# eric612/Mobilenet-YOLO-Pytorch

Hardware: AMD Instinct MI355X
Metric: images/sec MobileNetV2-YOLO 352x352 fwd+bwd @ bs256 (higher is better)
Workload: dtype f32; 1 GPU; MobileNetV2-YOLO 352x352 bs=256/GPU fwd+loss+bwd fp32 (BASELINE configs[1]); global_batch=256, parallelism=dp1

## Files before the change

### mobilenet-yolo-pytorch_amd/csrc/pwgemm.hip

```cpp
#include <map>
#include <mutex>

#include "pwgemm.h"
#include "x6.h"
#include "pwnt_kernel.h"

namespace mny {

static Nt2Kernel nt2_kernel(int TN, int XF, int BF = 0, int RED = 0, int X6 = 0, int RB = 0) {
    if (RED) return nt2_red_kernel(TN, XF, BF, RED, X6, RB);
#define MNY_K(T, XF_, BF_, RED_, X6_, RB_) case nt2_key(T, XF_, BF_, RED_, X6_, RB_): return (Nt2Kernel)pw_gemm_nt_dma_kernel<T, XF_, BF_, RED_, X6_, RB_>;
#define MNY_FWD(T, BF_, X6_) MNY_K(T, 0, BF_, 0, X6_, 0) MNY_K(T, 1, BF_, 0, X6_, 0) MNY_K(T, 2, BF_, 0, X6_, 0)
#define MNY_TN5(M_, ...) M_(1, __VA_ARGS__) M_(2, __VA_ARGS__) M_(3, __VA_ARGS__) M_(4, __VA_ARGS__) M_(5, __VA_ARGS__)
    switch (nt2_key(TN, XF, BF, RED, X6, RB)) {
        MNY_TN5(MNY_FWD, 0, 0) MNY_TN5(MNY_FWD, 0, 1) MNY_TN5(MNY_FWD, 0, 3) MNY_TN5(MNY_FWD, 1, 0)
    }
#undef MNY_TN5
#undef MNY_FWD
#undef MNY_K
    return nullptr;
}

struct Nt2Plan { int TN, n_tiles, m_tiles, gx, tiles_per_block, grid; size_t lds; };

// ... 14 lines not shown
    const Cut3Job jb = jobs[block_job[blockIdx.x]];
    const int nk = (jb.C + 15) / 16;
    const int64_t idx = (int64_t)(blockIdx.x - jb.block0) * 256 + threadIdx.x;
    if (idx >= (int64_t)jb.R * nk * 2) return;
    const int h = (int)(idx & 1);
    const int64_t rk = idx >> 1;
    const int kt = (int)(rk % nk);
    const int64_t row = rk / nk;
    float x[8];
#pragma unroll
    for (int e = 0; e < 8; ++e) {
        const int k = kt * 16 + (e < 4 ? 4 * h + e : 8 + 4 * h + (e - 4));
        x[e] = k < jb.C ? jb.src[row * jb.C + k] : 0.f;
    }
    bf16x8_t hh, mm, ll;
    x6_split(v4f_t{x[0], x[1], x[2], x[3]}, v4f_t{x[4], x[5], x[6], x[7]}, hh, mm, ll);
    const int64_t plane = (int64_t)jb.R * nk * 32;
    char* d = reinterpret_cast<char*>(jb.dst) + idx * 16;
    *reinterpret_cast<v4f_t*>(d) = __builtin_bit_cast(v4f_t, hh);
    *reinterpret_cast<v4f_t*>(d + plane) = __builtin_bit_cast(v4f_t, mm);
    *reinterpret_cast<v4f_t*>(d + 2 * plane) = __builtin_bit_cast(v4f_t, ll);
}

static int nt2_blocks_per_cu(int TN, int XF, size_t lds, int BF = 0) {
    static std::map<uint64_t, int> cache;
    static std::mutex mu;
    const uint64_t key = ((uint64_t)BF << 48) | ((uint64_t)TN << 40) | ((uint64_t)XF << 32) | (uint64_t)lds;
    std::lock_guard<std::mutex> lock(mu);
    auto it = cache.find(key);
    if (it != cache.end()) return it->second;
    int nb = 0;
    if (hipOccupancyMaxActiveBlocksPerMultiprocessor(&nb, (const void*)nt2_kernel(TN, XF, BF), 256, lds) != hipSuccess || nb < 1) nb = 1;
    if (nb > 8) nb = 8;
    cache[key] = nb;
    return nb;
}

static Nt2Plan nt2_plan(int64_t M, int K, int N, bool xf, int BF = 0, int tn_cap = 5) {
    Nt2Plan pl;
    int best = 1, best_pad = 1 << 30;
    for (int tn = tn_cap; tn >= 1; --tn) {
        int pad = (int)cdiv(N, 32 * tn) * 32 * tn;
        if (pad < best_pad) { best_pad = pad; best = tn; }
    }
    const int blocks_per_cu = nt2_blocks_per_cu(best, 1, nt2_lds(best, K, true, BF), BF);
    pl.TN = best;
    pl.n_tiles = (int)cdiv(N, 32 * best);
    pl.m_tiles = (int)cdiv(M, BM);
    int want = 256 * blocks_per_cu / pl.n_tiles;
    if (want < 8) want = 8;
    if (want > kMaxParts) want = kMaxParts;
    int gx = pl.m_tiles < want ? pl.m_tiles : want;
    pl.tiles_per_block = (int)cdiv(pl.m_tiles, gx);
    constexpr double min_ai = 100.0;
    const double ai = 2.0 * K * N / ((BF ? 2.0 : 4.0) * (K + N));
    if (ai >= min_ai) {
        const int t_min = pl.tiles_per_block;
        long best_cost = -1;
        int best_t = t_min, best_b = 0;
        for (int t = t_min; t <= 4 * t_min + 4 && t <= pl.m_tiles; ++t) {
            const int g = (int)cdiv(pl.m_tiles, t);
            const int nb = g * pl.n_tiles;
            if (nb < 256) break;
            const long cost = (long)cdiv(nb, 256) * t;
            if (best_cost < 0 || cost < best_cost || (cost == best_cost && nb > best_b)) { best_cost = cost; best_t = t; best_b = nb; }
        }
        pl.tiles_per_block = best_t;
    }
    pl.gx = (int)cdiv(pl.m_tiles, pl.tiles_per_block);
    pl.grid = (int)cdiv(pl.gx, 8) * 8 * pl.n_tiles;
    pl.lds = nt2_lds(best, K, xf, BF);
    return pl;
}

template <typename T>
__global__ void transpose_kernel(const float* __restrict__ src, T* __restrict__ dst, int R, int Cc, int Rp) {
    __shared__ float tile[32][33];
    const int bx = blockIdx.x * 32, by = blockIdx.y * 32;
    for (int j = threadIdx.y; j < 32; j += 8) {
        const int r = by + j, c = bx + threadIdx.x;
        tile[j][threadIdx.x] = (r < R && c < Cc) ? src[(int64_t)r * Cc + c] : 0.f;
    }
    __syncthreads();
    for (int j = threadIdx.y; j < 32; j += 8) {
        const int c = bx + j, r = by + threadIdx.x;
        if (r < Rp && c < Cc) st1(dst + (int64_t)c * Rp + r, r < R ? tile[threadIdx.x][j] : 0.f);
    }
}

}

using namespace mny;
static thread_local int g_pw_route = -1;
void mny::pw_set_last_route(int family) { g_pw_route = family; }

struct PwRoute {
    int family = MNY_ROUTE_TILE_V1;
    const char* why = nullptr;
    int parts = MNY_EINVAL;
    bool as_counted = true;
    int64_t Mf = 0;
    int wide_parts = 0;
    int x6 = 0;
    Nt2Plan p2{};
    size_t lds = 0;
};

static bool w6_pays(int K, int Nc) {
    constexpr double min_ai = 30.0;
    return !sw(SW_NO_W6) && 2.0 * K * Nc / (4.0 * (K + Nc)) >= min_ai;
}

static PwRoute pw_fwd_route(int bf, int64_t M, int K, int Nc, int in_act, bool view, bool bias, bool addend, bool planes) {
    PwRoute r;
    if (M <= 0 || K <= 0 || Nc <= 0) { r.why = "empty problem"; return r; }
    const bool v1 = sw(SW_GEMM_V1);
    const bool thin = pw_thin_ok(bf, 0, M, K, Nc);
    const bool wide = !bf && !thin && pw_wide_ok(M, K, Nc, false);
    auto family = [&](int act, bool has_bias, bool has_addend) {
        if (bf && pwt_ok(M, K, Nc, act, has_bias)) return MNY_ROUTE_WAVE16;
        if (thin) return MNY_ROUTE_THIN;
        if (wide && !has_bias && !has_addend && act != MNY_ACT_HSIGMOID) return MNY_ROUTE_WIDE;
        if ((K & (bf ? 7 : 3)) || v1) return MNY_ROUTE_TILE_V1;
        return !bf && nt_x6(M, K, Nc) ? MNY_ROUTE_DMA_X6 : MNY_ROUTE_DMA_F32;
    };
    r.family = family(in_act, bias, addend);
    const int plain = in_act == MNY_ACT_NONE && !bias && !addend ? r.family : family(MNY_ACT_NONE, false, false);
    r.as_counted = r.family == plain;
    if (planes && (bf || plain != MNY_ROUTE_DMA_X6 || pw_wide_ok(M, K, Nc, true) || !w6_pays(K, Nc))) r.why = "no pre-cut weight planes for this problem (mny_pw_w6_supported)";
    const bool xf = view || in_act != MNY_ACT_NONE;
    switch (r.family) {
        case MNY_ROUTE_WAVE16: r.parts = pwt_parts(M); return r;
        case MNY_ROUTE_THIN: r.parts = pw_thin_parts(M, K, Nc, 0); return r;
        case MNY_ROUTE_TILE_V1: r.parts = pw_v1_parts(M, K, Nc); return r;
        case MNY_ROUTE_WIDE:
            r.Mf = M & ~(int64_t)31;
            r.parts = r.wide_parts = pw_wide_parts(M, K, Nc, false);
            if (r.Mf == M) return r;
            r.p2 = nt2_plan(M - r.Mf, K, Nc, xf);
            r.x6 = nt_x6(M, K, Nc);
            r.parts += r.p2.gx;
            break;
        default:
            r.p2 = nt2_plan(M, K, Nc, xf, bf);
            r.x6 = r.family == MNY_ROUTE_DMA_X6;
            r.parts = r.p2.gx;
    }
    r.lds = r.p2.lds;
    size_t lds_max = 64 * 1024;
    if (planes) {
        r.x6 = 3;
#if MNY_W6_SWP
        r.lds = (size_t)(3 * BM * 16 + 3 * 32 * r.p2.TN * 24) * sizeof(float) + (xf ? 2 * cdiv(K, 16) * 16 * sizeof(float) : 0);
#endif
        lds_max = 96 * 1024;
    }
    if (!r.why && r.lds > lds_max) r.why = "K too large for the LDS scale cache";
    return r;
}

constexpr int kRedMaxTn = 4;
static PwRoute pw_dgrad_bnred_route(int bf, int64_t M, int K, int Nc, int act, bool addend, bool planes) {
    PwRoute r;
    if (M <= 0 || K <= 0 || Nc <= 0 || (K & (bf ? 7 : 3))) { r.why = "empty problem, or dy rows that are not 16-byte aligned"; return r; }
    const bool v1 = sw(SW_GEMM_V1), thin32 = pw_thin_ok(0, 1, M, K, Nc), wide = pw_wide_ok(M, K, Nc, true);
    r.x6 = !bf && nt_x6(M, K, Nc);
    bool tile = false;
    if (bf && pwt_ok(M, K, Nc, MNY_ACT_NONE, false)) {
        r.family = MNY_ROUTE_WAVE16;
        r.parts = pwt_parts(M);
    } else if (bf ? pw_thin_ok(1, 1, M, K, Nc) : thin32) {
        r.family = MNY_ROUTE_THIN;
        r.parts = pw_thin_parts(M, K, Nc, 1);
    } else if (!bf && wide) {
        r.family = MNY_ROUTE_WIDE;
        r.Mf = M & ~(int64_t)31;
        r.parts = r.wide_parts = pw_wide_parts(M, K, Nc, true);
        if (r.Mf != M) {
            r.p2 = nt2_plan(M - r.Mf, K, Nc, false, 0, kRedMaxTn);
            r.parts += r.p2.gx;
        }
    } else {
        r.family = v1 ? MNY_ROUTE_TILE_V1 : r.x6 ? MNY_ROUTE_DMA_X6 : MNY_ROUTE_DMA_F32;
        r.p2 = nt2_plan(M, K, Nc, false, bf, kRedMaxTn);
        r.parts = r.p2.gx;
        tile = true;
    }
    r.lds = r.p2.lds;
    if (act < MNY_ACT_NONE || act > MNY_ACT_HSIGMOID) r.why = "unknown activation";
    else if (v1) r.why = "MNY_GEMM_V1 is set";
    else if (K >= 512 && Nc >= 512) r.why = "matrix-pipe-bound: the reduce pass it would save is cheaper than the longer epilogue";
    else if (thin32 && act == MNY_ACT_HSIGMOID) r.why = "the short-reduction kernel knows the clamp family and h-swish (what units use)";
    else if (wide && act >= MNY_ACT_HSWISH) r.why = "the wide-output kernel's reduction form knows the clamp family (its h-swish builds spill)";
    else if (addend && tile && r.p2.TN > 3) r.why = "the addend form needs a column tile of <= 96 (mny_pw_dgrad_bnred_add_supported)";
    else if (planes && (bf || r.family != MNY_ROUTE_DMA_X6 || pw_wide_ok(M, K, Nc, false) || !w6_pays(K, Nc))) r.why = "no pre-cut weight planes for this problem (mny_pw_w6_supported)";
    else if (r.lds > (size_t)(planes ? 96 : 64) * 1024) r.why = "K too large";
    if (planes) r.x6 = 3;
    return r;
}

static PwRoute pw_lr_fix_route(int64_t M, int K, int r_act, bool red, bool view) {
    PwRoute r;
    if (M <= 0 || K <= 0 || (K & 3)) { r.why = "empty problem, or rows that are not 16-byte aligned"; return r; }
    if (red && pw_wide_fix_ok(M, K) && r_act < MNY_ACT_HSWISH) {
        r.family = MNY_ROUTE_WIDE;
        r.parts = pw_wide_fix_parts(M, K);
        return r;
    }
    r.p2 = nt2_plan(M, K, K, view, 0, 3);
    r.lds = r.p2.lds;
    r.x6 = nt_x6(M, K, K);
    r.family = r.x6 ? MNY_ROUTE_DMA_X6 : MNY_ROUTE_DMA_F32;
    r.parts = r.p2.gx;
    if (r.lds > 64 * 1024) r.why = "K too large";
    return r;
}

extern "C" int mny_pw_stat_parts(int64_t M, int K, int Nc) { return pw_fwd_route(0, M, K, Nc, MNY_ACT_NONE, false, false, false, false).parts; }
extern "C" int mny_pw_stat_parts_bf16(int64_t M, int K, int Nc) { return pw_fwd_route(1, M, K, Nc, MNY_ACT_NONE, false, false, false, false).parts; }

static int nt2_launch(const PwRoute& r, int XF, int BF, int RED, int RB, const Gemm2Args& g, hipStream_t st, const char* what) {
    const Nt2Kernel k = nt2_kernel(r.p2.TN, XF, BF, RED, r.x6, RB);
    if (!k) {
        set_error("%s: no kernel for a %d-column tile", what, 32 * r.p2.TN); return MNY_EUNSUPPORTED;
    }
    nt2_allow_lds(k, r.lds);
    hipLaunchKernelGGL(k, dim3(r.p2.grid), dim3(256), r.lds, st, g);
    return check_launch(what);
}

template <int BF>
static int pw_fwd_impl(const void* x, const float* in_scale, const float* in_shift, int in_act, const void* w, const float* bias, const void* addend,
                       void* y, float* stats, int64_t M, int K, int Nc, void* stream, bool planes = false) {
    MNY_REQUIRE(x && w && y, "pw_fwd: null pointer");
    MNY_REQUIRE(!(stats && bias), "pw_fwd: stats and bias are mutually exclusive");
    const PwRoute r = pw_fwd_route(BF, M, K, Nc, in_act, in_scale != nullptr, bias != nullptr, addend != nullptr, planes);
    MNY_REQUIRE(!r.why, "pw_fwd: M=%lld K=%d N=%d: %s", (long long)M, K, Nc, r.why);
    MNY_REQUIRE(!stats || r.as_counted, "pw_fwd: statistics with in_act=%d%s%s at M=%lld K=%d N=%d take another kernel family than mny_pw_stat_parts%s counted rows for",
                in_act, bias ? ", a bias" : "", addend ? ", an addend" : "", (long long)M, K, Nc, BF ? "_bf16" : "");
    g_pw_route = r.family;
    hipStream_t st = (hipStream_t)stream;
    switch (r.family) {
        case MNY_ROUTE_WAVE16: return pwt_launch(x, in_scale, in_shift, in_act, w, addend, y, stats, M, K, Nc, st);
        case MNY_ROUTE_THIN:
            return pw_thin_launch(BF, x, in_scale, in_shift, in_act, w, bias, addend, y, stats, M, K, Nc, 0, nullptr, nullptr, nullptr, nullptr, nullptr, 0, st);
        case MNY_ROUTE_TILE_V1: return pw_v1_launch(BF, x, in_scale, in_shift, in_act, w, bias, addend, y, stats, M, K, Nc, st);
        case MNY_ROUTE_WIDE: {
            const int rc = pw_wide_launch((const float*)x, in_scale, in_shift, in_act, (const float*)w, (float*)y, stats, r.Mf, K, Nc, nullptr, nullptr, nullptr, nullptr,
                                          nullptr, 0, nullptr, st);
            if (rc != 0 || r.Mf == M) return rc;
            if (stats) stats += (int64_t)r.wide_parts * 2 * Nc;
            x = (const float*)x + r.Mf * K; y = (float*)y + r.Mf * Nc; M -= r.Mf;
        }
    }
    Gemm2Args g{x, in_scale, in_shift, in_act, w, bias, addend, y, stats, M, K, Nc, r.p2.m_tiles, r.p2.tiles_per_block, r.p2.gx, r.p2.n_tiles,
                nullptr, nullptr, nullptr, nullptr, nullptr, 0};
    const int XF = !in_scale && in_act == MNY_ACT_NONE ? 0 : (in_act == MNY_ACT_HSWISH ? 2 : 1);
    return nt2_launch(r, XF, BF, 0, 0, g, st, "pw_gemm_nt_dma_kernel");
}
extern "C" int mny_pw_fwd(const float* x, const float* in_scale, const float* in_shift, int in_act, const float* w,
                          const float* bias, const float* addend, float* y, float* stats, int64_t M, int K, int Nc,
                          void* stream) {
    return pw_fwd_impl<0>(x, in_scale, in_shift, in_act, w, bias, addend, y, stats, M, K, Nc, stream);
}
extern "C" int mny_pw_fwd_bf16(const void* x, const float* in_scale, const float* in_shift, int in_act, const void* w,
                               const float* bias, const void* addend, void* y, float* stats, int64_t M, int K, int Nc,
                               void* stream) {
    return pw_fwd_impl<1>(x, in_scale, in_shift, in_act, w, bias, addend, y, stats, M, K, Nc, stream);
}

template <int BF>
static int pw_dgrad_bnred_impl(const void* dy, const void* wT, void* dx, const void* y, const float* scale, const float* shift, int act,
                               const float* mean, const float* invstd, float* red, int64_t M, int K, int Nc, void* stream, const void* addend = nullptr,
                               bool planes = false) {
    MNY_REQUIRE(dy && wT && dx && y && scale && shift && mean && invstd && red, "pw_dgrad_bnred: null pointer");
    const PwRoute r = pw_dgrad_bnred_route(BF, M, K, Nc, act, addend != nullptr, planes);
    MNY_REQUIRE(!r.why, "pw_dgrad_bnred: unsupported problem M=%lld K=%d N=%d act=%d: %s (see mny_pw_dgrad_bnred_supported)", (long long)M, K, Nc, act, r.why);
    g_pw_route = r.family;
    hipStream_t st = (hipStream_t)stream;
    switch (r.family) {
        case MNY_ROUTE_WAVE16: return pwt_launch(dy, nullptr, nullptr, MNY_ACT_NONE, wT, addend, dx, red, M, K, Nc, st, y, scale, shift, mean, invstd, act);
        case MNY_ROUTE_THIN:
            return pw_thin_launch(BF, dy, nullptr, nullptr, MNY_ACT_NONE, wT, nullptr, addend, dx, red, M, K, Nc, addend ? 2 : 1, y, scale, shift, mean, invstd, act, st);
        case MNY_ROUTE_WIDE: {
            const int rc = pw_wide_launch((const float*)dy, nullptr, nullptr, MNY_ACT_NONE, (const float*)wT, (float*)dx, red, r.Mf, K, Nc, (const float*)y, scale, shift,
                                          mean, invstd, act, (const float*)addend, st);
            if (rc != 0 || r.Mf == M) return rc;
            red += (int64_t)r.wide_parts * 2 * Nc;
            dy = (const float*)dy + r.Mf * K; dx = (float*)dx + r.Mf * Nc; y = (const float*)y + r.Mf * Nc;
            if (addend) addend = (const float*)addend + r.Mf * Nc;
            M -= r.Mf;
        }
    }
    Gemm2Args g{dy, nullptr, nullptr, MNY_ACT_NONE, wT, nullptr, addend, dx, red, M, K, Nc, r.p2.m_tiles, r.p2.tiles_per_block, r.p2.gx, r.p2.n_tiles,
                y, scale, shift, mean, invstd, act};
    return nt2_launch(r, 0, BF, addend ? 2 : 1, 0, g, st, "pw_gemm_nt_dma_kernel<RED>");
}
extern "C" int mny_pw_dgrad_bnred_supported(int64_t M, int K, int Nc, int act) { return !pw_dgrad_bnred_route(0, M, K, Nc, act, false, false).why; }
extern "C" int mny_pw_dgrad_bnred_parts(int64_t M, int K, int Nc) { return pw_dgrad_bnred_route(0, M, K, Nc, MNY_ACT_NONE, false, false).parts; }
extern "C" int mny_pw_dgrad_bnred(const float* dy, const float* wT, float* dx, const float* y, const float* scale, const float* shift, int act,
                                  const float* mean, const float* invstd, float* red, int64_t M, int K, int Nc, void* stream) {
    return pw_dgrad_bnred_impl<0>(dy, wT, dx, y, scale, shift, act, mean, invstd, red, M, K, Nc, stream);
}
extern "C" int mny_pw_dgrad_bnred_add_supported(int64_t M, int K, int Nc, int act) { return !pw_dgrad_bnred_route(0, M, K, Nc, act, true, false).why; }
extern "C" int mny_pw_dgrad_bnred_add_supported_bf16(int64_t M, int K, int Nc, int act) { return !pw_dgrad_bnred_route(1, M, K, Nc, act, true, false).why; }
extern "C" int mny_pw_dgrad_bnred_add(const float* dy, const float* wT, const float* addend, float* dx, const float* y, const float* scale, const float* shift,
// ... 113 lines not shown
```

### mobilenet-yolo-pytorch_amd/csrc/pwnt_kernel.h

```cpp
#pragma once
#include <type_traits>

#include "common.h"
#include "dma_zero.h"
#include "x6.h"

namespace mny {

constexpr int BM = 128;

struct Gemm2Args {
    const void* A; const float* in_scale; const float* in_shift; int in_act;
    const void* B; const float* bias; const void* addend; void* C; float* stats;
    int64_t M; int K; int N;
    int m_tiles, tiles_per_block, gx, n_tiles;
    const void* rY; const float* r_scale; const float* r_shift; const float* r_mean; const float* r_invstd; int r_act;
};

#ifndef MNY_W6_GROUP
#define MNY_W6_GROUP 4
#endif
#ifndef MNY_W6_SWP
#define MNY_W6_SWP 1
#endif
template <int TN, int XF, int BF, int RED = 0, int X6 = 0, int RB = 0>
__global__ __launch_bounds__(256) __attribute__((amdgpu_waves_per_eu((X6 == 3 && RED == 0 && MNY_W6_SWP) ? 2 : 3, 8))) void pw_gemm_nt_dma_kernel(Gemm2Args p) {
    using T = typename std::conditional<BF != 0, bf16_t, float>::type;
    constexpr int EPC = BF ? 8 : 4;
    constexpr int BKE = 4 * EPC;
    const T* pA = (const T*)p.A;
    const T* pB = (const T*)p.B;
    const T* pAdd = (const T*)p.addend;
    T* pC = (T*)p.C;
    constexpr int BN = 32 * TN, BKD = 16, S = 3;
    constexpr int A_ST = BM * BKD, B_ST = X6 == 3 ? BN * 24 : BN * BKD;
    constexpr int NA = BM / 16, NB = X6 == 3 ? 3 * TN : BN / 16, NL = NA + NB;
    constexpr int LPW = (NL + 3) / 4;
    constexpr bool SWP = X6 == 3 && RED == 0 && MNY_W6_SWP != 0;
    constexpr int SB = X6 == 3 ? (SWP ? 3 : 2) : S;
    constexpr int NA_W = NA / 4;
    static_assert(NA % 4 == 0 && NA_W < LPW, "slot split");
    extern __shared__ __attribute__((aligned(16))) float smem[];
    float* const sA = smem;
    float* const sB = smem + S * A_ST;
    float* sScale = sB + SB * B_ST;

    const int bid = blockIdx.x, xcd = bid & 7, local = bid >> 3;
    const int y = local % p.n_tiles, x = (local / p.n_tiles) * 8 + xcd;
    if (x >= p.gx) return;
    const int n0 = y * BN;

    const int tid = threadIdx.x, lane = tid & 63;
    const int wv = __builtin_amdgcn_readfirstlane(tid >> 6);
    const int lrow = lane & 31, khalf = lane >> 5;
    const int swz = (lrow >> 2) & 3;
    const int nk = (p.K + BKE - 1) / BKE;
    const int Kpad = nk * BKE;
    float* sShift = sScale + Kpad;
    const float slope = act_slope(p.in_act), hi = act_hi(p.in_act);
    if (XF != 0) {
        const bool has_xf = p.in_scale != nullptr;
        for (int k = tid; k < Kpad; k += 256) {
            sScale[k] = (k < p.K) ? (has_xf ? p.in_scale[k] : 1.f) : 0.f;
            sShift[k] = (k < p.K && has_xf) ? p.in_shift[k] : 0.f;
        }
    }
    const int mt_begin = x * p.tiles_per_block;
    const int mt_end = min(mt_begin + p.tiles_per_block, p.m_tiles);
    const int total = (mt_end - mt_begin) * nk;

    const int drow = lane >> 2;
    const int dk = ((lane & 3) ^ ((drow >> 2) & 3)) * EPC;
    int d_lds[LPW], d_row0[LPW];
    bool d_isA[LPW];
    const T* d_bptr[LPW];
#pragma unroll
    for (int i = 0; i < LPW; ++i) {
        int j = wv + 4 * i;
        if (j >= NL) j = NL - 1;
        d_isA[i] = j < NA;
        d_row0[i] = (d_isA[i] ? j : j - NA) * 16;
        d_lds[i] = d_isA[i] ? j * 256 : (j - NA) * 256;
        if constexpr (X6 == 3) {
            const int jb = d_isA[i] ? 0 : j - NA;
            const int pl = jb / TN, u = jb - pl * TN;
            int n = n0 + u * 32 + (lane & 31);
            if (n >= p.N) n = p.N - 1;
            d_lds[i] = d_isA[i] ? j * 256 : jb * 256;
            d_bptr[i] = reinterpret_cast<const T*>(reinterpret_cast<const char*>(p.B) + ((int64_t)pl * p.N + n) * nk * 32 + (lane >> 5) * 16);
        } else {
            int n = n0 + d_row0[i] + drow;
            if (n >= p.N) n = p.N - 1;
            d_bptr[i] = pB + (int64_t)n * p.K + dk;
        }
    }
    const T* zero_src = reinterpret_cast<const T*>(&mny_zero16);
    const bool ragged_k = (p.K % BKE) != 0;

    const T* d_cur[LPW];
    int d_step[LPW];
#pragma unroll
    for (int i = 0; i < LPW; ++i) d_step[i] = d_isA[i] ? BKE : (X6 == 3 ? 32 / (int)sizeof(T) : BKE);
    auto seat = [&](int mt) {
#pragma unroll
        for (int i = 0; i < LPW; ++i) {
            if (d_isA[i]) {
                int m = mt * BM + d_row0[i] + drow;
                if (m >= (int)p.M) m = (int)p.M - 1;
                d_cur[i] = pA + (int64_t)m * p.K + dk;
            } else {
                d_cur[i] = d_bptr[i];
            }
        }
    };
    auto issue_part = [&](int kt, float* stage, int i0, int i1) {
#pragma unroll
        for (int i = 0; i < LPW; ++i) {
            if (i < i0 || i >= i1) continue;
            const T* src = d_cur[i];
            if (ragged_k) {
                const bool kout = kt == nk - 1 && kt * BKE + dk >= p.K;
                if (kout) src = d_isA[i] ? d_cur[i] - (kt * BKE + dk) : (X6 == 3 ? src : zero_src);
            }
            d_cur[i] += d_step[i];
            __builtin_amdgcn_global_load_lds((const __attribute__((address_space(1))) void*)src,
                                             (__attribute__((address_space(3))) void*)(stage + d_lds[i]), 16, 0, 0);
        }
    };
    auto issue_a = [&](int kt, int slot) { issue_part(kt, sA + slot * A_ST, 0, NA_W); };
    auto issue_b = [&](int kt, int slot) { issue_part(kt, sB + slot * B_ST, NA_W, LPW); };

    f32x16 acc[TN];
#pragma unroll
    for (int t = 0; t < TN; ++t)
#pragma unroll
        for (int r = 0; r < 16; ++r) acc[t][r] = 0.f;
    float s1[TN], s2[TN];
#pragma unroll
    for (int t = 0; t < TN; ++t) { s1[t] = 0.f; s2[t] = 0.f; }

    auto compute = [&](int kt, int slot, int slot_b) {
        const float* stA = sA + slot * A_ST;
        const float* stB = sB + slot_b * B_ST;
        const float* a_row = stA + (wv * 32 + lrow) * BKD;
        if constexpr (BF != 0) {
#pragma unroll
            for (int kc = 0; kc < 2; ++kc) {
                const int chunk = kc * 2 + khalf;
                v4u_t au = lds_read_u4(a_row + ((chunk ^ swz) << 2));
                v4u_t bu[TN];
#pragma unroll
                for (int u = 0; u < TN; ++u) bu[u] = lds_read_u4(stB + (u * 32 + lrow) * BKD + ((chunk ^ swz) << 2));
                v4f_t sc0, sc1, sh0, sh1;
                if (XF != 0) {
                    const int kbase = kt * BKE + chunk * 8;
                    sc0 = lds_read_f4(sScale + kbase); sc1 = lds_read_f4(sScale + kbase + 4);
                    sh0 = lds_read_f4(sShift + kbase); sh1 = lds_read_f4(sShift + kbase + 4);
                }
                MNY_LGKM_WAIT(au);
#pragma unroll
                for (int u = 0; u < TN; ++u) MNY_LGKM_DEP(bu[u]);
                if (XF != 0) {
                    MNY_LGKM_DEP(sc0); MNY_LGKM_DEP(sc1); MNY_LGKM_DEP(sh0); MNY_LGKM_DEP(sh1);
                    float z[8] = {__uint_as_float(au.x << 16), __uint_as_float(au.x & 0xffff0000u), __uint_as_float(au.y << 16),
                                  __uint_as_float(au.y & 0xffff0000u), __uint_as_float(au.z << 16), __uint_as_float(au.z & 0xffff0000u),
                                  __uint_as_float(au.w << 16), __uint_as_float(au.w & 0xffff0000u)};
                    const float scv[8] = {sc0.x, sc0.y, sc0.z, sc0.w, sc1.x, sc1.y, sc1.z, sc1.w};
                    const float shv[8] = {sh0.x, sh0.y, sh0.z, sh0.w, sh1.x, sh1.y, sh1.z, sh1.w};
#pragma unroll
                    for (int e = 0; e < 8; ++e) {
                        const float zz = fmaf(z[e], scv[e], shv[e]);
                        z[e] = XF == 1 ? __builtin_amdgcn_fmed3f(zz, slope * zz, hi) : zz * __builtin_amdgcn_fmed3f(zz + 3.f, 0.f, 6.f) * (1.f / 6.f);
                    }
                    au = v4u_t{pack_bf16x2(z[0], z[1]), pack_bf16x2(z[2], z[3]), pack_bf16x2(z[4], z[5]), pack_bf16x2(z[6], z[7])};
                }
                const bf16x8_t a8 = __builtin_bit_cast(bf16x8_t, au);
// ... 93 lines not shown
                    af.x = z0 * fminf(fmaxf(z0 + 3.f, 0.f), 6.f) * (1.f / 6.f); af.y = z1 * fminf(fmaxf(z1 + 3.f, 0.f), 6.f) * (1.f / 6.f);
                    af.z = z2 * fminf(fmaxf(z2 + 3.f, 0.f), 6.f) * (1.f / 6.f); af.w = z3 * fminf(fmaxf(z3 + 3.f, 0.f), 6.f) * (1.f / 6.f);
                }
            }
#pragma unroll
            for (int u = 0; u < TN; ++u) acc[u] = __builtin_amdgcn_mfma_f32_32x32x2f32(af.x, bf[u].x, acc[u], 0, 0, 0);
#pragma unroll
            for (int u = 0; u < TN; ++u) acc[u] = __builtin_amdgcn_mfma_f32_32x32x2f32(af.y, bf[u].y, acc[u], 0, 0, 0);
#pragma unroll
            for (int u = 0; u < TN; ++u) acc[u] = __builtin_amdgcn_mfma_f32_32x32x2f32(af.z, bf[u].z, acc[u], 0, 0, 0);
#pragma unroll
            for (int u = 0; u < TN; ++u) acc[u] = __builtin_amdgcn_mfma_f32_32x32x2f32(af.w, bf[u].w, acc[u], 0, 0, 0);
        }
    };

    const int quad = lrow >> 2, jq = lane & 3;
    const bool nvec = (p.N & 3) == 0;
    auto epilogue = [&](int mt) {
        const int64_t m0 = (int64_t)mt * BM;
#pragma unroll
        for (int u = 0; u < TN; ++u) {
            const int colq = n0 + u * 32 + quad * 4;
            const bool cok = colq < p.N;
            float4 bv = f4zero();
            if (p.bias && cok) {
                if (nvec) bv = ld4(p.bias + colq);
                else {
                    bv.x = p.bias[colq];
                    if (colq + 1 < p.N) bv.y = p.bias[colq + 1];
                    if (colq + 2 < p.N) bv.z = p.bias[colq + 2];
                    if (colq + 3 < p.N) bv.w = p.bias[colq + 3];
                }
            }
            if (RED) {
                const int col = n0 + u * 32 + lrow;
                const bool ccol = col < p.N;
                const int cc = ccol ? col : 0;
                const float rsc = p.r_scale[cc], rsh = p.r_shift[cc], rmu = p.r_mean[cc], ris = p.r_invstd[cc];
                float rbias = 0.f;
                if constexpr (RB != 0) rbias = p.bias[cc];
                const float rslope = act_slope(p.r_act), rhi = act_hi(p.r_act);
                const int64_t rbase = m0 + wv * 32 + 4 * khalf;
                const int rows_left = (int)max((int64_t)0, min((int64_t)64, p.M - rbase));
                const T* ybase = (const T*)p.rY + (rows_left > 0 ? rbase : 0) * p.N + cc;
                const T* abase = RED == 2 ? pAdd + (rows_left > 0 ? rbase : 0) * p.N + cc : nullptr;
#pragma unroll
                for (int gq = 0; gq < 4; ++gq) {
                    float yv[4], av[4] = {0.f, 0.f, 0.f, 0.f};
#pragma unroll
                    for (int j = 0; j < 4; ++j) yv[j] = ld1(ybase + (ccol && 8 * gq + j < rows_left ? 8 * gq + j : 0) * p.N);
                    if (RED == 2) {
#pragma unroll
                        for (int j = 0; j < 4; ++j) av[j] = ld1(abase + (ccol && 8 * gq + j < rows_left ? 8 * gq + j : 0) * p.N);
                    }
#pragma unroll
                    for (int j = 0; j < 4; ++j) {
                        const float z = fmaf(yv[j], rsc, rsh);
                        const float dact = p.r_act >= MNY_ACT_HSWISH ? act_bwd(z, p.r_act) : (z > 0.f ? 1.f : rslope) * (z < rhi ? 1.f : 0.f);
                        const float dz = stored<T>(RB != 0 ? acc[u][gq * 4 + j] + rbias + av[j] : acc[u][gq * 4 + j] + av[j]) * dact;
                        if (ccol && 8 * gq + j < rows_left) { s1[u] += dz; s2[u] = fmaf(dz, (yv[j] - rmu) * ris, s2[u]); }
                    }
                    __builtin_amdgcn_sched_barrier(0);
                }
            } else if (p.stats) {
                const bool ccol = n0 + u * 32 + lrow < p.N;
                if (m0 + BM <= p.M) {
                    v2f a1 = v2f{0.f, 0.f}, a2 = v2f{0.f, 0.f};
#pragma unroll
                    for (int r = 0; r < 16; r += 2) {
                        const v2f q = v2f{stored<T>(acc[u][r]), stored<T>(acc[u][r + 1])};
                        a1 += q;
                        a2 = __builtin_elementwise_fma(q, q, a2);
                    }
                    if (ccol) { s1[u] += a1.x + a1.y; s2[u] += a2.x + a2.y; }
                } else {
#pragma unroll
                    for (int r = 0; r < 16; ++r) {
                        const int64_t row = m0 + wv * 32 + (r & 3) + 8 * (r >> 2) + 4 * khalf;
                        const float q = stored<T>(acc[u][r]);
                        if (ccol && row < p.M) { s1[u] += q; s2[u] = fmaf(q, q, s2[u]); }
                    }
                }
            }
#pragma unroll
            for (int gq = 0; gq < 4; ++gq) {
                float r0 = acc[u][gq * 4 + 0], r1 = acc[u][gq * 4 + 1], r2 = acc[u][gq * 4 + 2], r3 = acc[u][gq * 4 + 3];
                {
                    const bool odd = lane & 1;
                    const float xa = odd ? r0 : r1, xb = odd ? r2 : r3;
                    const float ya = __builtin_bit_cast(float, __builtin_amdgcn_mov_dpp(__builtin_bit_cast(int, xa), 0xB1, 0xF, 0xF, true));
                    const float yb = __builtin_bit_cast(float, __builtin_amdgcn_mov_dpp(__builtin_bit_cast(int, xb), 0xB1, 0xF, 0xF, true));
                    if (odd) { r0 = ya; r2 = yb; } else { r1 = ya; r3 = yb; }
                }
                {
                    const bool hi2 = lane & 2;
                    const float xa = hi2 ? r0 : r2, xb = hi2 ? r1 : r3;
                    const float ya = __builtin_bit_cast(float, __builtin_amdgcn_mov_dpp(__builtin_bit_cast(int, xa), 0x4E, 0xF, 0xF, true));
                    const float yb = __builtin_bit_cast(float, __builtin_amdgcn_mov_dpp(__builtin_bit_cast(int, xb), 0x4E, 0xF, 0xF, true));
                    if (hi2) { r0 = ya; r1 = yb; } else { r2 = ya; r3 = yb; }
                }
                const int64_t row = m0 + wv * 32 + 8 * gq + 4 * khalf + jq;
                if (cok && row < p.M) {
                    float4 v = make_float4(r0, r1, r2, r3);
                    if (p.bias) { v.x += bv.x; v.y += bv.y; v.z += bv.z; v.w += bv.w; }
                    if (nvec) {
                        if (pAdd) add4(v, ld4(pAdd + row * p.N + colq));
                        if (sizeof(T) == 2) st4(pC + row * p.N + colq, v); else st4_stream(pC + row * p.N + colq, v);
                    } else {
                        T* dst = pC + row * p.N + colq;
                        const T* ad = pAdd ? pAdd + row * p.N + colq : nullptr;
                        st1(dst, v.x + (ad ? ld1(ad) : 0.f));
                        if (colq + 1 < p.N) st1(dst + 1, v.y + (ad ? ld1(ad + 1) : 0.f));
                        if (colq + 2 < p.N) st1(dst + 2, v.z + (ad ? ld1(ad + 2) : 0.f));
                        if (colq + 3 < p.N) st1(dst + 3, v.w + (ad ? ld1(ad + 3) : 0.f));
                    }
                }
#pragma unroll
                for (int i = 0; i < 4; ++i) acc[u][gq * 4 + i] = 0.f;
                __builtin_amdgcn_sched_barrier(0);
            }
        }
    };

    int c_mt = mt_begin, c_kt = 0, c_slot = 0, c_slot_b = 0;
    auto consume = [&]() {
        compute(c_kt, c_slot, X6 != 3 ? c_slot : c_slot_b);
        if (++c_kt == nk) { epilogue(c_mt); c_kt = 0; ++c_mt; }
        if (++c_slot == S) c_slot = 0;
        c_slot_b ^= 1;
    };
    if constexpr (X6 != 3) {
        int i_mt = mt_begin, i_kt = 0, i_slot = 0;
        seat(mt_begin);
        auto issue_next = [&]() {
            issue_a(i_kt, i_slot); issue_b(i_kt, i_slot);
            if (++i_kt == nk) { i_kt = 0; ++i_mt; if (i_mt < mt_end) seat(i_mt); }
            if (++i_slot == S) i_slot = 0;
        };
        const int pre = total < S - 1 ? total : S - 1;
        for (int t = 0; t < pre; ++t) issue_next();
        const int steady = total - pre;
        for (int t = 0; t < steady; ++t) {
            wait_vmcnt<LPW*(S - 2)>();
            __builtin_amdgcn_s_barrier();
            issue_next();
            consume();
        }
        for (int t = 0; t < pre; ++t) {
            wait_vmcnt<0>();
            __builtin_amdgcn_s_barrier();
            consume();
        }
    } else if constexpr (SWP) {
        int a_mt = mt_begin, a_kt = 0, a_slot = 0, a_n = 0;
        int b_mt = mt_begin, b_kt = 0, b_slot = 0, b_n = 0;
        auto seat_part = [&](int mt, bool part_a) {
#pragma unroll
            for (int i = 0; i < LPW; ++i) {
                if ((i < NA_W) != part_a) continue;
                if (part_a) {
                    int m = mt * BM + d_row0[i] + drow;
                    if (m >= (int)p.M) m = (int)p.M - 1;
                    d_cur[i] = pA + (int64_t)m * p.K + dk;
                } else {
                    d_cur[i] = d_bptr[i];
                }
            }
        };
        seat_part(mt_begin, true); seat_part(mt_begin, false);
        auto next_a = [&]() {
            issue_a(a_kt, a_slot); ++a_n;
            if (++a_kt == nk) { a_kt = 0; ++a_mt; if (a_mt < mt_end) seat_part(a_mt, true); }
            if (++a_slot == S) a_slot = 0;
        };
        auto next_b = [&]() {
            issue_b(b_kt, b_slot); ++b_n;
            if (++b_kt == nk) { b_kt = 0; ++b_mt; if (b_mt < mt_end) seat_part(b_mt, false); }
            if (++b_slot == SB) b_slot = 0;
        };
        const unsigned oA0 = lds_off(sA + (wv * 32 + lrow) * BKD + ((khalf ^ swz) << 2));
        const unsigned oA1 = lds_off(sA + (wv * 32 + lrow) * BKD + (((2 + khalf) ^ swz) << 2));
        const unsigned oB = lds_off(sB + lane * 4);
        const unsigned oS = lds_off(sScale + khalf * 4);
        const unsigned shift_off = (unsigned)Kpad * 4u;
        bf16x8_t qh, qm, ql;
        int p_kt = 0, p_slot = 0;
        int m_slot_b = 0;
        auto step = [&](auto prep_c, auto mma_c) -> bool {
            constexpr bool PREP = decltype(prep_c)::value, MMA = decltype(mma_c)::value;
            constexpr int NPIECE = 24, NISSUE = MMA ? 6 * TN : 1;
            v4f_t a0, a1, sc0, sc1, sh0, sh1;
            float z[8];
            v2f r1[4], r2[4];
            v4u_t nhu, nmu, nlu;
            auto piece = [&](auto pc) {
                constexpr int P = decltype(pc)::value;
                if constexpr (PREP) {
                    if constexpr (P < 8) {
                        const float av = P < 4 ? a0[P & 3] : a1[P & 3];
                        if constexpr (XF != 0) {
                            const float zz = fmaf(av, P < 4 ? sc0[P & 3] : sc1[P & 3], P < 4 ? sh0[P & 3] : sh1[P & 3]);
                            z[P] = XF == 1 ? __builtin_amdgcn_fmed3f(zz, slope * zz, hi) : zz * __builtin_amdgcn_fmed3f(zz + 3.f, 0.f, 6.f) * (1.f / 6.f);
                        } else {
                            z[P] = av;
                        }
                        asm volatile("" : "+v"(z[P]));
                    } else if constexpr (P < 16) {
                        constexpr int i = (P - 8) >> 1;
                        if constexpr (((P - 8) & 1) == 0) {
                            const v2f a = v2f{z[2 * i], z[2 * i + 1]};
                            const v2f ah = v2f{__uint_as_float(__float_as_uint(a.x) & 0xffff0000u), __uint_as_float(__float_as_uint(a.y) & 0xffff0000u)};
                            r1[i] = a - ah;
                            asm volatile("" : "+v"(r1[i]));
                        } else {
                            const v2f b = r1[i];
                            const v2f bh = v2f{__uint_as_float(__float_as_uint(b.x) & 0xffff0000u), __uint_as_float(__float_as_uint(b.y) & 0xffff0000u)};
                            r2[i] = b - bh;
                            asm volatile("" : "+v"(r2[i]));
                        }
                    } else if constexpr (P < 22) {
                        constexpr int q = P - 16, w = q >> 1, d = (q & 1) * 2;
                        auto pk = [](float lo, float hi_) { return __builtin_amdgcn_perm(__float_as_uint(hi_), __float_as_uint(lo), 0x07060302u); };
                        unsigned t0, t1;
                        if constexpr (w == 0) { t0 = pk(z[2 * d], z[2 * d + 1]); t1 = pk(z[2 * d + 2], z[2 * d + 3]); }
                        if constexpr (w == 1) { t0 = pk(r1[d].x, r1[d].y); t1 = pk(r1[d + 1].x, r1[d + 1].y); }
                        if constexpr (w == 2) { t0 = pk(r2[d].x, r2[d].y); t1 = pk(r2[d + 1].x, r2[d + 1].y); }
                        asm volatile("" : "+v"(t0), "+v"(t1));
                        if constexpr (w == 0) { nhu[d] = t0; nhu[d + 1] = t1; }
                        if constexpr (w == 1) { nmu[d] = t0; nmu[d + 1] = t1; }
                        if constexpr (w == 2) { nlu[d] = t0; nlu[d + 1] = t1; }
                    }
                }
            };
            auto pieces_of = [&](auto ic) {
                constexpr int I = decltype(ic)::value;
                static_for<0, NPIECE>([&](auto pc) {
                    constexpr int P = decltype(pc)::value;
                    if constexpr (P * NISSUE / NPIECE == I) piece(pc);
                });
            };
            if constexpr (!MMA) {
                const unsigned bA = (unsigned)p_slot * (A_ST * 4);
                a0 = lds_read_f4_at<0>(oA0 + bA); a1 = lds_read_f4_at<0>(oA1 + bA);
                if constexpr (XF != 0) {
                    const unsigned bS = oS + (unsigned)p_kt * (BKD * 4), bH = bS + shift_off;
                    sc0 = lds_read_f4_at<0>(bS); sc1 = lds_read_f4_at<32>(bS); sh0 = lds_read_f4_at<0>(bH); sh1 = lds_read_f4_at<32>(bH);
                    asm volatile("s_waitcnt lgkmcnt(0)" : "+v"(a0), "+v"(a1), "+v"(sc0), "+v"(sc1), "+v"(sh0), "+v"(sh1));
                } else {
                    asm volatile("s_waitcnt lgkmcnt(0)" : "+v"(a0), "+v"(a1));
                }
                pieces_of(std::integral_constant<int, 0>{});
            } else {
                const unsigned bB = oB + (unsigned)m_slot_b * (B_ST * 4);
                v4f_t PH[TN], PM[TN], PL[TN];
                constexpr int NPREP = PREP ? (XF != 0 ? 6 : 2) : 0;
                constexpr int G0 = TN <= MNY_W6_GROUP ? TN : (TN + 1) / 2;
                auto rdH = [&](auto uc) { constexpr int u = decltype(uc)::value; PH[u] = lds_read_f4_at<u * 1024>(bB); };
                auto rdM = [&](auto uc) { constexpr int u = decltype(uc)::value; PM[u] = lds_read_f4_at<(TN + u) * 1024>(bB); };
                auto rdL = [&](auto uc) { constexpr int u = decltype(uc)::value; PL[u] = lds_read_f4_at<(2 * TN + u) * 1024>(bB); };
                auto tie = [&](auto uc, v4f_t* P_) { constexpr int u = decltype(uc)::value; asm volatile("" : "+v"(P_[u])); };
                auto group = [&](auto u0c, auto gsc, auto firstc) {
                    constexpr int u0 = decltype(u0c)::value, gs = decltype(gsc)::value;
                    constexpr bool first = decltype(firstc)::value;
                    constexpr bool more = u0 + gs < TN;
                    constexpr int I0 = 6 * u0;
                    if constexpr (first) {
                        static_for<u0, u0 + gs>(rdH);
                        if constexpr (PREP) {
                            const unsigned bA = (unsigned)p_slot * (A_ST * 4);
                            a0 = lds_read_f4_at<0>(oA0 + bA); a1 = lds_read_f4_at<0>(oA1 + bA);
                            if constexpr (XF != 0) {
                                const unsigned bS = oS + (unsigned)p_kt * (BKD * 4), bH = bS + shift_off;
                                sc0 = lds_read_f4_at<0>(bS); sc1 = lds_read_f4_at<32>(bS); sh0 = lds_read_f4_at<0>(bH); sh1 = lds_read_f4_at<32>(bH);
                            }
                        }
                        static_for<u0, u0 + gs>(rdL);
                        static_for<u0, u0 + gs>(rdM);
                        asm volatile("s_waitcnt lgkmcnt(%0)" :: "n"(NPREP + 2 * gs) : "memory");
                        static_for<u0, u0 + gs>([&](auto uc) { tie(uc, PH); });
                    } else {
                        asm volatile("s_waitcnt lgkmcnt(0)" ::: "memory");
                        static_for<u0, u0 + gs>([&](auto uc) { tie(uc, PH); tie(uc, PL); tie(uc, PM); });
                    }
                    auto prod = [&](auto kc, const bf16x8_t& A_, v4f_t* P_) {
                        constexpr int k = decltype(kc)::value;
                        static_for<0, gs>([&](auto jc) {
                            constexpr int j = decltype(jc)::value, u = u0 + j, IA = I0 + k * gs + j;
                            acc[u] = __builtin_amdgcn_mfma_f32_32x32x16_bf16(A_, __builtin_bit_cast(bf16x8_t, P_[u]), acc[u], 0, 0, 0);
                            if constexpr (PREP && first && k == 0 && j == 0) {
                                if constexpr (XF != 0) asm volatile("s_waitcnt lgkmcnt(%6)" : "+v"(a0), "+v"(a1), "+v"(sc0), "+v"(sc1), "+v"(sh0), "+v"(sh1) : "n"(2 * gs));
                                else asm volatile("s_waitcnt lgkmcnt(%2)" : "+v"(a0), "+v"(a1) : "n"(2 * gs));
                            }
                            pieces_of(std::integral_constant<int, IA>{});
                            __builtin_amdgcn_sched_barrier(0);
                        });
                    };
                    prod(std::integral_constant<int, 0>{}, ql, PH);
                    if constexpr (first) {
                        asm volatile("s_waitcnt lgkmcnt(%0)" :: "n"(gs) : "memory");
                        static_for<u0, u0 + gs>([&](auto uc) { tie(uc, PL); });
                    }
                    prod(std::integral_constant<int, 1>{}, qh, PL);
                    if constexpr (first) {
                        asm volatile("s_waitcnt lgkmcnt(0)" ::: "memory");
                        static_for<u0, u0 + gs>([&](auto uc) { tie(uc, PM); });
                        if constexpr (more) { static_for<u0 + gs, TN>(rdH); static_for<u0 + gs, TN>(rdL); static_for<u0 + gs, TN>(rdM); }
                    }
                    prod(std::integral_constant<int, 2>{}, qm, PM);
                    prod(std::integral_constant<int, 3>{}, qm, PH);
                    prod(std::integral_constant<int, 4>{}, qh, PM);
                    prod(std::integral_constant<int, 5>{}, qh, PH);
                };
                group(std::integral_constant<int, 0>{}, std::integral_constant<int, G0>{}, std::true_type{});
                if constexpr (G0 < TN) group(std::integral_constant<int, G0>{}, std::integral_constant<int, TN - G0>{}, std::false_type{});
            }
            bool fin = false;
            if constexpr (MMA) {
                if (++c_kt == nk) { c_kt = 0; fin = true; }
                if (++m_slot_b == SB) m_slot_b = 0;
            }
            if constexpr (PREP) {
                qh = __builtin_bit_cast(bf16x8_t, nhu); qm = __builtin_bit_cast(bf16x8_t, nmu); ql = __builtin_bit_cast(bf16x8_t, nlu);
                if (++p_kt == nk) p_kt = 0;
                if (++p_slot == S) p_slot = 0;
            }
            return fin;
        };
        if (total > 0) { next_a(); next_b(); }
        if (total > 1) next_a();
        if (total > 0) {
            wait_vmcnt<NA_W>();
            if (total == 1) wait_vmcnt<0>();
            __builtin_amdgcn_s_barrier();
            if (b_n < total) next_b();
            if (a_n < total) next_a();
            step(std::true_type{}, std::false_type{});
            for (int t = 1; t < total; ++t) {
                if (t + 1 < total) wait_vmcnt<NA_W>(); else wait_vmcnt<0>();
                __builtin_amdgcn_s_barrier();
                if (b_n < total) next_b();
                if (a_n < total) next_a();
                if (step(std::true_type{}, std::true_type{})) { epilogue(c_mt); ++c_mt; }
            }
            step(std::false_type{}, std::true_type{});
            epilogue(c_mt);
        }
    } else {
        int a_mt = mt_begin, a_kt = 0, a_slot = 0, a_n = 0;
        int b_mt = mt_begin, b_kt = 0, b_slot = 0, b_n = 0;
        auto seat_part = [&](int mt, bool part_a) {
#pragma unroll
            for (int i = 0; i < LPW; ++i) {
                if ((i < NA_W) != part_a) continue;
                if (part_a) {
                    int m = mt * BM + d_row0[i] + drow;
                    if (m >= (int)p.M) m = (int)p.M - 1;
                    d_cur[i] = pA + (int64_t)m * p.K + dk;
                } else {
                    d_cur[i] = d_bptr[i];
                }
            }
        };
        seat_part(mt_begin, true); seat_part(mt_begin, false);
        auto next_a = [&]() {
            issue_a(a_kt, a_slot); ++a_n;
            if (++a_kt == nk) { a_kt = 0; ++a_mt; if (a_mt < mt_end) seat_part(a_mt, true); }
            if (++a_slot == S) a_slot = 0;
        };
        auto next_b = [&]() {
            issue_b(b_kt, b_slot); ++b_n;
            if (++b_kt == nk) { b_kt = 0; ++b_mt; if (b_mt < mt_end) seat_part(b_mt, false); }
            b_slot ^= 1;
        };
        if (total > 0) { next_a(); next_b(); }
        if (total > 1) next_a();
        for (int t = 0; t < total; ++t) {
            if (t + 1 < total) wait_vmcnt<NA_W>(); else wait_vmcnt<0>();
            __builtin_amdgcn_s_barrier();
            if (b_n < total) next_b();
            if (a_n < total) next_a();
            consume();
        }
    }

    if (p.stats) {
        wait_vmcnt<0>();
        __syncthreads();
        float* red = smem;
#pragma unroll
        for (int u = 0; u < TN; ++u) {
            const float a = s1[u] + __shfl_xor(s1[u], 32);
            const float b = s2[u] + __shfl_xor(s2[u], 32);
            if (khalf == 0) {
                red[(wv * BN + u * 32 + lrow) * 2 + 0] = a;
                red[(wv * BN + u * 32 + lrow) * 2 + 1] = b;
            }
        }
        __syncthreads();
        if (tid < BN && n0 + tid < p.N) {
            float a = 0.f, b = 0.f;
#pragma unroll
            for (int w = 0; w < 4; ++w) { a += red[(w * BN + tid) * 2]; b += red[(w * BN + tid) * 2 + 1]; }
            p.stats[(int64_t)x * 2 * p.N + n0 + tid] = a;
            p.stats[(int64_t)x * 2 * p.N + p.N + n0 + tid] = b;
        }
    }
}

typedef void (*Nt2Kernel)(Gemm2Args);
static constexpr int nt2_key(int TN, int XF, int BF, int RED, int X6, int RB) { return ((((TN * 3 + XF) * 2 + BF) * 3 + RED) * 4 + X6) * 2 + RB; }
Nt2Kernel nt2_red_kernel(int TN, int XF, int BF, int RED, int X6, int RB);

}
```

Before: 7244 images/s.

## Restructure weight-plane GEMM pipeline with offset-based DMA issue and ring-slot tracking

Rewrites the software-pipelined X6 weight-plane path of the pointwise GEMM so its global-to-LDS loads use a base pointer plus precomputed 32-bit per-lane offsets instead of per-lane 64-bit pointers. Slot and k-index bookkeeping moves into a shared rotating ring state, with an optional compile-time unrolled variant that turns slot indices into constant LDS offsets. The aim is to cut VGPR pressure and per-iteration scalar/vector address arithmetic in the hot loop. Because of the 32-bit offsets, the route planner now rejects weight planes of 4 GiB or more.

```diff
diff --git a/mobilenet-yolo-pytorch_amd/csrc/pwgemm.hip b/mobilenet-yolo-pytorch_amd/csrc/pwgemm.hip
--- a/mobilenet-yolo-pytorch_amd/csrc/pwgemm.hip
+++ b/mobilenet-yolo-pytorch_amd/csrc/pwgemm.hip
@@ -190,6 +190,7 @@
         r.x6 = 3;
 #if MNY_W6_SWP
         r.lds = (size_t)(3 * BM * 16 + 3 * 32 * r.p2.TN * 24) * sizeof(float) + (xf ? 2 * cdiv(K, 16) * 16 * sizeof(float) : 0);
+        if (!r.why && 3.0 * Nc * cdiv(K, 16) * 32.0 >= 4294967296.0) r.why = "weight planes of 4 GiB or more";
 #endif
         lds_max = 96 * 1024;
     }
diff --git a/mobilenet-yolo-pytorch_amd/csrc/pwnt_kernel.h b/mobilenet-yolo-pytorch_amd/csrc/pwnt_kernel.h
--- a/mobilenet-yolo-pytorch_amd/csrc/pwnt_kernel.h
+++ b/mobilenet-yolo-pytorch_amd/csrc/pwnt_kernel.h
@@ -22,6 +22,9 @@
 #endif
 #ifndef MNY_W6_SWP
 #define MNY_W6_SWP 1
+#endif
+#ifndef MNY_W6_RING_UNROLL
+#define MNY_W6_RING_UNROLL 0
 #endif
 template <int TN, int XF, int BF, int RED = 0, int X6 = 0, int RB = 0>
 __global__ __launch_bounds__(256) __attribute__((amdgpu_waves_per_eu((X6 == 3 && RED == 0 && MNY_W6_SWP) ? 2 : 3, 8))) void pw_gemm_nt_dma_kernel(Gemm2Args p) {
@@ -421,31 +424,63 @@
             consume();
         }
     } else if constexpr (SWP) {
-        int a_mt = mt_begin, a_kt = 0, a_slot = 0, a_n = 0;
-        int b_mt = mt_begin, b_kt = 0, b_slot = 0, b_n = 0;
-        auto seat_part = [&](int mt, bool part_a) {
-#pragma unroll
-            for (int i = 0; i < LPW; ++i) {
-                if ((i < NA_W) != part_a) continue;
-                if (part_a) {
-                    int m = mt * BM + d_row0[i] + drow;
-                    if (m >= (int)p.M) m = (int)p.M - 1;
-                    d_cur[i] = pA + (int64_t)m * p.K + dk;
-                } else {
-                    d_cur[i] = d_bptr[i];
-                }
-            }
-        };
-        seat_part(mt_begin, true); seat_part(mt_begin, false);
-        auto next_a = [&]() {
-            issue_a(a_kt, a_slot); ++a_n;
-            if (++a_kt == nk) { a_kt = 0; ++a_mt; if (a_mt < mt_end) seat_part(a_mt, true); }
-            if (++a_slot == S) a_slot = 0;
-        };
-        auto next_b = [&]() {
-            issue_b(b_kt, b_slot); ++b_n;
-            if (++b_kt == nk) { b_kt = 0; ++b_mt; if (b_mt < mt_end) seat_part(b_mt, false); }
-            if (++b_slot == SB) b_slot = 0;
+        constexpr int NB_W = LPW - NA_W;
+        constexpr int STB = BKE * (int)sizeof(T);
+        const char* const gA = reinterpret_cast<const char*>(p.A);
+        const char* const gB = reinterpret_cast<const char*>(p.B);
+        int a_lds[NA_W], b_lds[NB_W];
+        unsigned a_off[NA_W], b_off[NB_W];
+        int a_row[NA_W];
+#pragma unroll
+        for (int i = 0; i < NA_W; ++i) { a_lds[i] = (wv + 4 * i) * 256; a_row[i] = (wv + 4 * i) * 16 + drow; a_off[i] = 0; }
+#pragma unroll
+        for (int i = 0; i < NB_W; ++i) {
+            int jb = wv + 4 * (NA_W + i) - NA;
+            if (jb >= NB) jb = NB - 1;
+            const int pl = jb / TN, u = jb - pl * TN;
+            int n = n0 + u * 32 + (lane & 31);
+            if (n >= p.N) n = p.N - 1;
+            b_lds[i] = jb * 256;
+            b_off[i] = ((unsigned)pl * (unsigned)p.N + (unsigned)n) * ((unsigned)nk * 32u) + (unsigned)(lane >> 5) * 16u;
+        }
+        const int64_t a_tile_bytes = (int64_t)BM * p.K * (int64_t)sizeof(T);
+        const char* a_tile = gA + (int64_t)mt_begin * a_tile_bytes;
+        const char* a_src = a_tile;
+        int a_rows = (int)p.M - mt_begin * BM;
+        const unsigned a_quiet = (unsigned)((ragged_k ? nk - 1 : nk) - 1);
+        auto dma = [&](const char* base, unsigned off, float* dst) {
+            __builtin_amdgcn_global_load_lds((const __attribute__((address_space(1))) void*)(base + off), (__attribute__((address_space(3))) void*)dst, 16, 0, 0);
+        };
+        auto issue_a_at = [&](auto slot, int k) {
+            float* const ring = sA + (int)slot * A_ST;
+            if (__builtin_expect((unsigned)(k - 1) >= a_quiet, 0)) {
+                if (k == 0) {
+                    a_src = a_tile;
+                    a_tile += a_tile_bytes;
+#pragma unroll
+                    for (int i = 0; i < NA_W; ++i) a_off[i] = (unsigned)min(a_row[i], a_rows - 1) * ((unsigned)p.K * (unsigned)sizeof(T)) + (unsigned)dk * (unsigned)sizeof(T);
+                    a_rows -= BM;
+                }
+                if (ragged_k && k == nk - 1) {
+                    const bool kout = k * BKE + dk >= p.K;
+                    a_src -= (int64_t)k * STB;
+#pragma unroll
+                    for (int i = 0; i < NA_W; ++i) a_off[i] = kout ? a_off[i] - (unsigned)dk * (unsigned)sizeof(T) : a_off[i] + (unsigned)k * STB;
+                }
+            }
+#pragma unroll
+            for (int i = 0; i < NA_W; ++i) dma(a_src, a_off[i], ring + a_lds[i]);
+            a_src += STB;
+        };
+        auto issue_b_at = [&](auto slot, int k) {
+            float* const ring = sB + (int)slot * B_ST;
+            const char* base = gB + (unsigned)k * 32u;
+            asm("" : "+s"(base));
+#pragma unroll
+            for (int i = 0; i < NB_W; ++i) {
+                asm volatile("" : "+v"(b_off[i]));
+                dma(base, b_off[i], ring + b_lds[i]);
+            }
         };
         const unsigned oA0 = lds_off(sA + (wv * 32 + lrow) * BKD + ((khalf ^ swz) << 2));
         const unsigned oA1 = lds_off(sA + (wv * 32 + lrow) * BKD + (((2 + khalf) ^ swz) << 2));
@@ -453,11 +488,18 @@
         const unsigned oS = lds_off(sScale + khalf * 4);
         const unsigned shift_off = (unsigned)Kpad * 4u;
         bf16x8_t qh, qm, ql;
-        int p_kt = 0, p_slot = 0;
-        int m_slot_b = 0;
-        auto step = [&](auto prep_c, auto mma_c) -> bool {
+        auto rd = [](auto offc, auto stridec, unsigned base, auto slot) -> v4f_t {
+            constexpr int OFF = decltype(offc)::value, STRIDE = decltype(stridec)::value;
+            using SlotT = decltype(slot);
+            if constexpr (std::is_integral<SlotT>::value) return lds_read_f4_at<OFF>(base + (unsigned)slot * STRIDE);
+            else return lds_read_f4_at<OFF + SlotT::value * STRIDE>(base);
+        };
+        auto step = [&](auto prep_c, auto mma_c, auto p_slot, int p_kt, auto m_slot_b) {
             constexpr bool PREP = decltype(prep_c)::value, MMA = decltype(mma_c)::value;
             constexpr int NPIECE = 24, NISSUE = MMA ? 6 * TN : 1;
+            constexpr std::integral_constant<int, 0> o0{};
+            constexpr std::integral_constant<int, A_ST * 4> strideA{};
+            constexpr std::integral_constant<int, B_ST * 4> strideB{};
             v4f_t a0, a1, sc0, sc1, sh0, sh1;
             float z[8];
             v2f r1[4], r2[4];
@@ -509,8 +551,7 @@
                 });
             };
             if constexpr (!MMA) {
-                const unsigned bA = (unsigned)p_slot * (A_ST * 4);
-                a0 = lds_read_f4_at<0>(oA0 + bA); a1 = lds_read_f4_at<0>(oA1 + bA);
+                a0 = rd(o0, strideA, oA0, p_slot); a1 = rd(o0, strideA, oA1, p_slot);
                 if constexpr (XF != 0) {
                     const unsigned bS = oS + (unsigned)p_kt * (BKD * 4), bH = bS + shift_off;
                     sc0 = lds_read_f4_at<0>(bS); sc1 = lds_read_f4_at<32>(bS); sh0 = lds_read_f4_at<0>(bH); sh1 = lds_read_f4_at<32>(bH);
@@ -520,13 +561,12 @@
                 }
                 pieces_of(std::integral_constant<int, 0>{});
             } else {
-                const unsigned bB = oB + (unsigned)m_slot_b * (B_ST * 4);
                 v4f_t PH[TN], PM[TN], PL[TN];
                 constexpr int NPREP = PREP ? (XF != 0 ? 6 : 2) : 0;
                 constexpr int G0 = TN <= MNY_W6_GROUP ? TN : (TN + 1) / 2;
-                auto rdH = [&](auto uc) { constexpr int u = decltype(uc)::value; PH[u] = lds_read_f4_at<u * 1024>(bB); };
-                auto rdM = [&](auto uc) { constexpr int u = decltype(uc)::value; PM[u] = lds_read_f4_at<(TN + u) * 1024>(bB); };
-                auto rdL = [&](auto uc) { constexpr int u = decltype(uc)::value; PL[u] = lds_read_f4_at<(2 * TN + u) * 1024>(bB); };
+                auto rdH = [&](auto uc) { constexpr int u = decltype(uc)::value; PH[u] = rd(std::integral_constant<int, u * 1024>{}, strideB, oB, m_slot_b); };
+                auto rdM = [&](auto uc) { constexpr int u = decltype(uc)::value; PM[u] = rd(std::integral_constant<int, (TN + u) * 1024>{}, strideB, oB, m_slot_b); };
+                auto rdL = [&](auto uc) { constexpr int u = decltype(uc)::value; PL[u] = rd(std::integral_constant<int, (2 * TN + u) * 1024>{}, strideB, oB, m_slot_b); };
                 auto tie = [&](auto uc, v4f_t* P_) { constexpr int u = decltype(uc)::value; asm volatile("" : "+v"(P_[u])); };
                 auto group = [&](auto u0c, auto gsc, auto firstc) {
                     constexpr int u0 = decltype(u0c)::value, gs = decltype(gsc)::value;
@@ -536,8 +576,7 @@
                     if constexpr (first) {
                         static_for<u0, u0 + gs>(rdH);
                         if constexpr (PREP) {
-                            const unsigned bA = (unsigned)p_slot * (A_ST * 4);
-                            a0 = lds_read_f4_at<0>(oA0 + bA); a1 = lds_read_f4_at<0>(oA1 + bA);
+                            a0 = rd(o0, strideA, oA0, p_slot); a1 = rd(o0, strideA, oA1, p_slot);
                             if constexpr (XF != 0) {
                                 const unsigned bS = oS + (unsigned)p_kt * (BKD * 4), bH = bS + shift_off;
                                 sc0 = lds_read_f4_at<0>(bS); sc1 = lds_read_f4_at<32>(bS); sh0 = lds_read_f4_at<0>(bH); sh1 = lds_read_f4_at<32>(bH);
@@ -583,35 +622,52 @@
                 group(std::integral_constant<int, 0>{}, std::integral_constant<int, G0>{}, std::true_type{});
                 if constexpr (G0 < TN) group(std::integral_constant<int, G0>{}, std::integral_constant<int, TN - G0>{}, std::false_type{});
             }
-            bool fin = false;
-            if constexpr (MMA) {
-                if (++c_kt == nk) { c_kt = 0; fin = true; }
-                if (++m_slot_b == SB) m_slot_b = 0;
-            }
-            if constexpr (PREP) {
-                qh = __builtin_bit_cast(bf16x8_t, nhu); qm = __builtin_bit_cast(bf16x8_t, nmu); ql = __builtin_bit_cast(bf16x8_t, nlu);
-                if (++p_kt == nk) p_kt = 0;
-                if (++p_slot == S) p_slot = 0;
-            }
+            if constexpr (PREP) { qh = __builtin_bit_cast(bf16x8_t, nhu); qm = __builtin_bit_cast(bf16x8_t, nmu); ql = __builtin_bit_cast(bf16x8_t, nlu); }
+        };
+        static_assert(S == 3 && SB == 3, "both rings are three slots deep");
+        int k0 = 0, k1 = nk > 1 ? 1 : 0, k2 = nk > 2 ? 2 : 0;
+        auto advance = [&]() { k0 = k1; k1 = k2; k2 = k2 + 1 == nk ? 0 : k2 + 1; };
+        auto next_slot = [](auto s) {
+            if constexpr (std::is_integral<decltype(s)>::value) return s == 2 ? 0 : s + 1;
+            else return std::integral_constant<int, (decltype(s)::value + 1) % 3>{};
+        };
+        auto stage = [&](auto r, int t) {
+            const auto rn = next_slot(r);
+            const auto rp = next_slot(rn);
+            if (t + 1 < total) wait_vmcnt<NA_W>(); else wait_vmcnt<0>();
+            __builtin_amdgcn_s_barrier();
+            if (t + 1 < total) issue_b_at(rn, k1);
+            if (t + 2 < total) issue_a_at(rp, k2);
+            step(std::true_type{}, std::true_type{}, r, k0, rp);
+            const bool fin = k0 == 0;
+            advance();
             return fin;
         };
-        if (total > 0) { next_a(); next_b(); }
-        if (total > 1) next_a();
         if (total > 0) {
+            issue_a_at(std::integral_constant<int, 0>{}, k0);
+            issue_b_at(std::integral_constant<int, 0>{}, k0);
+            if (total > 1) issue_a_at(std::integral_constant<int, 1>{}, k1);
             wait_vmcnt<NA_W>();
             if (total == 1) wait_vmcnt<0>();
             __builtin_amdgcn_s_barrier();
-            if (b_n < total) next_b();
-            if (a_n < total) next_a();
-            step(std::true_type{}, std::false_type{});
+            if (total > 1) issue_b_at(std::integral_constant<int, 1>{}, k1);
+            if (total > 2) issue_a_at(std::integral_constant<int, 2>{}, k2);
+            step(std::true_type{}, std::false_type{}, std::integral_constant<int, 0>{}, k0, 0);
+            advance();
+            int r = 1;
             for (int t = 1; t < total; ++t) {
-                if (t + 1 < total) wait_vmcnt<NA_W>(); else wait_vmcnt<0>();
-                __builtin_amdgcn_s_barrier();
-                if (b_n < total) next_b();
-                if (a_n < total) next_a();
-                if (step(std::true_type{}, std::true_type{})) { epilogue(c_mt); ++c_mt; }
-            }
-            step(std::false_type{}, std::true_type{});
+                bool fin;
+#if MNY_W6_RING_UNROLL
+                if (r == 1) { fin = stage(std::integral_constant<int, 1>{}, t); r = 2; }
+                else if (r == 2) { fin = stage(std::integral_constant<int, 2>{}, t); r = 0; }
+                else { fin = stage(std::integral_constant<int, 0>{}, t); r = 1; }
+#else
+                fin = stage(r, t);
+                r = next_slot(r);
+#endif
+                if (fin) { epilogue(c_mt); ++c_mt; }
+            }
+            step(std::false_type{}, std::true_type{}, 0, 0, r == 0 ? 2 : r - 1);
             epilogue(c_mt);
         }
     } else {
```

New measurement: 7269 images/s (median of 3 runs). About the same (+0.3%).
